# qq456cvb/VoteNet

Measured on AMD Instinct MI355X. Metric: SUN RGB-D 20k-pt scenes/sec (fwd+bwd), higher is better.
Workload: dtype f32

## Files before the change

votenet_amd/csrc/pool_bwd.hip:

```cpp
#include "mlp_types.h"
#include <mutex>
#include <set>

namespace votenet {

bool wgrad_fast_launch(int mode, const MlpIn &d, long rows, int cin, int cout, const float *dz, const BnSrc &bs, int bsrc, float *dw,
                       hipStream_t st, float *scratch);
void wgrad_reduce(int nslice, long pstride, long e0, long e1, const float *part, float *dw, hipStream_t st);

static inline int pb_grid(long total, int block, int cap)
{
    long g = (total + block - 1) / block;
    if (g > cap) g = cap;
    return (int)(g < 1 ? 1 : g);
}

__global__ __launch_bounds__(256) void bn_bwd_reduce_zsel_kernel(long groups, int c, const float *__restrict__ gout,
                                                                 const float *__restrict__ zsel, const float *__restrict__ scale,
                                                                 const float *__restrict__ shift, const float *__restrict__ mean,
                                                                 const float *__restrict__ var, float eps, int relu,
                                                                 double *__restrict__ sums, CoefTail tail)
{
    __shared__ float sh1[4][64], sh2[4][64];
    const int cx = threadIdx.x & 63, ry = threadIdx.x >> 6;
// ... 738 lines not shown
        for (int d = 0; d < D; d++) {
            if (c0 + (long)d * stride >= G) break;
            const long c = c0 + team + (long)d * stride;
            const bool live = c < G;
            float(*xt)[K][LD] = xs[buf];
            bool kept[NP];
#pragma unroll
            for (int j = 0; j < NP; j++) {
                kept[j] = n_row[d][j] >= 0;
                if (!kept[j]) continue;
#pragma unroll
                for (int h = 0; h < NL; h++) {
                    float4 v = nxt[d][j][h];
                    v.x = fmaxf(v.x * sc.x + sh.x, fl);
                    v.y = fmaxf(v.y * sc.y + sh.y, fl);
                    v.z = fmaxf(v.z * sc.z + sh.z, fl);
                    v.w = fmaxf(v.w * sc.w + sh.w, fl);
                    *reinterpret_cast<float4 *>(&xt[j][(tid + h * 256) / Q][q * 4]) = v;
                }
            }
            float gg = live ? n_g[d] : 0.0f;
            const float zz = n_z[d], w31 = n_w[d];
            const int ar = n_a[d];
            const long cn = c + (long)D * stride;
            fetch(d, cn < G ? cn : (live ? c : G - 1));
            __syncthreads();
            if (own) {
                if (relu && !(zz * cS + cH > 0.0f)) gg = 0.0f;
                const float v = cA * gg;
                const int pj = ar >> 4;
                const bool there = pj == 0 ? kept[0] : pj == 1 ? kept[1] : pj == 2 ? kept[2] : kept[3];
                if (v != 0.0f && there) {
                    const float4 *row = reinterpret_cast<const float4 *>(&xt[pj][ar & (K - 1)][0]);
#pragma unroll
                    for (int i0 = 0; i0 < Q; i0 += 8) {
                        float4 a[8];
#pragma unroll
                        for (int i = 0; i < 8; i++) a[i] = row[i0 + i];
                        asm volatile("" ::: "memory");
#pragma unroll
                        for (int i = 0; i < 8; i++) {
                            acc[4 * (i0 + i)] += a[i].x * v;
                            acc[4 * (i0 + i) + 1] += a[i].y * v;
                            acc[4 * (i0 + i) + 2] += a[i].z * v;
                            acc[4 * (i0 + i) + 3] += a[i].w * v;
                        }
                    }
                }
            }
            if (live && tid >= 256 - CIN) {
                const int jc = tid - (256 - CIN);
#pragma unroll
                for (int j = 0; j < NP; j++) {
                    if (!kept[j]) continue;
#pragma unroll 8
                    for (int r = (j == 0 ? 1 : 0); r < K; r++) csum += xt[j][r][jc];
                }
                csum += w31 * xt[0][0][jc];
            }
            buf ^= 1;
        }
    }
    if (TEAMS > 1) {
        __syncthreads();
        float *comb = sparse_smem;
        if (team == 1) {
            if (own) {
#pragma unroll
                for (int i = 0; i < CIN; i++) comb[(size_t)i * cout + tid] = acc[i];
            }
            if (tid >= 256 - CIN) comb[(size_t)CIN * cout + tid - (256 - CIN)] = csum;
        }
        __syncthreads();
        if (team == 1) return;
        if (own) {
#pragma unroll
            for (int i = 0; i < CIN; i++) acc[i] += comb[(size_t)i * cout + tid];
        }
        if (tid >= 256 - CIN) csum += comb[(size_t)CIN * cout + tid - (256 - CIN)];
    }
    if (own) {
#pragma unroll
        for (int i = 0; i < CIN; i++) unsafeAtomicAdd(&dw[(size_t)i * cout + tid], acc[i]);
    }
    if (tid >= 256 - CIN) unsafeAtomicAdd(&colsum[tid - (256 - CIN)], csum);
}

__global__ __launch_bounds__(256) void pool_wgrad_finish_kernel(int cin, int cout, const float *__restrict__ gram,
                                                                const float *__restrict__ colsum, const float *__restrict__ w,
                                                                const float *__restrict__ bias, const float *__restrict__ coef,
                                                                float *__restrict__ dw)
{
    __shared__ float Gs[16][33], Ws[32][17];
    const int tx = threadIdx.x & 15, ty = threadIdx.x >> 4;
    const int j0 = blockIdx.y * 16, c0 = blockIdx.x * 16;
    float acc = 0.0f;
    for (int i0 = 0; i0 < cin; i0 += 32) {
        for (int e = threadIdx.x; e < 16 * 32; e += 256) {
            const int r = e >> 5, ii = e & 31;
            Gs[r][ii] = (j0 + r < cin && i0 + ii < cin) ? gram[(size_t)(j0 + r) * cin + i0 + ii] : 0.0f;
            const int wr = e >> 4, wc = e & 15;
            Ws[wr][wc] = (i0 + wr < cin && c0 + wc < cout) ? w[(size_t)(i0 + wr) * cout + c0 + wc] : 0.0f;
        }
        __syncthreads();
#pragma unroll 8
        for (int ii = 0; ii < 32; ii++) acc += Gs[ty][ii] * Ws[ii][tx];
        __syncthreads();
    }
    const int j = j0 + ty, c = c0 + tx;
    if (j < cin && c < cout) {
        const float Cc = coef[2 * cout + c];
        dw[(size_t)j * cout + c] += Cc * acc + colsum[j] * (coef[cout + c] + Cc * (bias ? bias[c] : 0.0f));
    }
}

}

using namespace votenet;

extern "C" int votenet_pool_backward_supported(int cin, int cout, int k)
{
    return k == 64 && ((cin == 128 && (cout == 256 || cout == 128)) || (cin == 64 && cout == 128));
}

static int g_zsel_groups = 32, g_zsel_cap = 256;
extern "C" void votenet_debug_zsel_grid(int groups_per_wg, int cap)
{
    VN_DEBUG_GATE();
    g_zsel_groups = groups_per_wg > 0 ? groups_per_wg : 32;
    g_zsel_cap = cap > 0 ? cap : 256;
}
extern "C" int votenet_bn_backward_reduce_pool(long groups, int c, const float *gout, const float *zsel, const float *scale,
                                               const float *shift, const float *mean, const float *var, float eps, int relu,
                                               double *sums, const votenet_coef_tail *tail, void *stream)
{
    VN_REQUIRE(groups > 0 && c > 0, "bn_backward_reduce_pool expects groups > 0, c > 0");
    VN_REQUIRE(gout && zsel && scale && shift && mean && var && sums, "bn_backward_reduce_pool: null buffer");
    VN_REQUIRE(!tail || (tail->ticket && tail->gamma && tail->coef && tail->rows > 0), "bn_backward_reduce_pool: incomplete coefficient tail");
    const int ny = (c + 63) / 64;
    hipLaunchKernelGGL(bn_bwd_reduce_zsel_kernel, dim3(pb_grid(groups, g_zsel_groups, g_zsel_cap / ny), ny), dim3(256), 0, as_stream(stream), groups,
                       c, gout, zsel, scale, shift, mean, var, eps, relu, sums, to_tail(tail));
    return check_launch("bn_backward_reduce_pool");
}

static int pool_dgrad_prepare_launch(int cin, int cout, const float *w, const float *bias, const float *coef, float *mmat, float *cvec,
                                     void *image, void *stream, float *h2_ascale = nullptr, float *h2_unscale = nullptr)
{
    VN_REQUIRE(cin > 0 && w && coef && mmat && cvec, "pool_dgrad_prepare: bad arguments");
    VN_REQUIRE((cout == 128 || cout == 256) && (uintptr_t)w % 16 == 0, "pool_dgrad_prepare: cout must be 128 or 256 (got %d), w 16-byte aligned", cout);
    VN_REQUIRE(image == nullptr || (cin % 16 == 0 && (uintptr_t)image % 16 == 0), "pool_dgrad_prepare_split: cin %% 16 == 0 and a 16-byte aligned image");
    const dim3 grid((cin + 15) / 16, (cin + 15) / 16);
    unsigned *img = static_cast<unsigned *>(image);
    if (cout == 256)
        hipLaunchKernelGGL(pool_dgrad_prepare_kernel<256>, grid, dim3(256), 0, as_stream(stream), cin, w, bias, coef, mmat, cvec, img, h2_ascale, h2_unscale);
    else
        hipLaunchKernelGGL(pool_dgrad_prepare_kernel<128>, grid, dim3(256), 0, as_stream(stream), cin, w, bias, coef, mmat, cvec, img, h2_ascale, h2_unscale);
    return check_launch("pool_dgrad_prepare");
}
extern "C" int votenet_pool_dgrad_prepare(int cin, int cout, const float *w, const float *bias, const float *coef, float *mmat,
                                          float *cvec, void *stream)
{
    return pool_dgrad_prepare_launch(cin, cout, w, bias, coef, mmat, cvec, nullptr, stream);
}
extern "C" int votenet_pool_dgrad_prepare_h2(int cin, int cout, const float *w, const float *bias, const float *coef, float *mmat,
                                             float *cvec, void *image, float *ascale, float *unscale, void *stream)
{
    VN_REQUIRE(image != nullptr && ascale != nullptr && unscale != nullptr, "pool_dgrad_prepare_h2: null image / scale vectors");
    return pool_dgrad_prepare_launch(cin, cout, w, bias, coef, mmat, cvec, image, stream, ascale, unscale);
}
extern "C" int votenet_pool_dgrad_prepare_split(int cin, int cout, const float *w, const float *bias, const float *coef, float *mmat,
                                                float *cvec, void *image, void *stream)
{
    VN_REQUIRE(image != nullptr, "pool_dgrad_prepare_split: null image");
    return pool_dgrad_prepare_launch(cin, cout, w, bias, coef, mmat, cvec, image, stream);
}

static int g_scatter_reverse = 0;
extern "C" void votenet_debug_scatter_reverse(int on) { VN_DEBUG_GATE(); g_scatter_reverse = on ? 1 : 0; }
static int g_scatter_nwv = 16;
extern "C" void votenet_debug_scatter_waves(int n) { VN_DEBUG_GATE(); g_scatter_nwv = n == 12 ? 12 : 16; }
static int g_scatter_wgs = 0;
extern "C" void votenet_debug_scatter_workgroups(int n) { VN_DEBUG_GATE(); g_scatter_wgs = n > 0 ? n : 0; }
static int g_scatter_form = 1;
extern "C" void votenet_debug_scatter_form(int form) { VN_DEBUG_GATE(); g_scatter_form = form ? 1 : 0; }
static int pool_dgrad_scatter_launch(long groups, int k, int cin, int cout, const float *gout, const int *argmax, const float *zsel,
                                     const float *coef, int relu, const float *wT, float *da, const float *below_z,
                                     const float *below_scale, const float *below_shift, const float *below_mean, const float *below_var,
                                     float eps, int below_relu, double *below_sums, const votenet_coef_tail *below_tail, const int *hc,
                                     const float *wh, int G, void *stream, const int *nh_dev = nullptr);
extern "C" int votenet_pool_dgrad_scatter(long groups, int k, int cin, int cout, const float *gout, const int *argmax,
                                          const float *zsel, const float *coef, int relu, const float *wT, float *da,
                                          const float *below_z, const float *below_scale, const float *below_shift,
                                          const float *below_mean, const float *below_var, float eps, int below_relu,
                                          double *below_sums, const votenet_coef_tail *below_tail, void *stream)
{
    VN_REQUIRE(!below_tail || (below_z && below_tail->ticket && below_tail->gamma && below_tail->coef && below_tail->rows > 0),
               "pool_dgrad_scatter: incomplete coefficient tail");
    VN_REQUIRE(groups > 0 && gout && argmax && zsel && coef && wT && da, "pool_dgrad_scatter: bad arguments");
    VN_REQUIRE(votenet_pool_backward_supported(cin, cout, k), "pool_dgrad_scatter: unsupported shape cin=%d cout=%d k=%d", cin, cout, k);
    VN_REQUIRE((uintptr_t)wT % 16 == 0, "pool_dgrad_scatter: wT must be 16-byte aligned");
    VN_REQUIRE(!below_z || (below_scale && below_shift && below_mean && below_var && below_sums),
               "pool_dgrad_scatter: below_z given without the layer's BatchNorm vectors / sums");
    return pool_dgrad_scatter_launch(groups, k, cin, cout, gout, argmax, zsel, coef, relu, wT, da, below_z, below_scale, below_shift, below_mean,
                                     below_var, eps, below_relu, below_sums, below_tail, nullptr, nullptr, 0, stream);
}

extern "C" int votenet_pool_dgrad_scatter_half(long nh, int G, int cin, int cout, const float *gout, const int *argmax, const float *zsel,
                                               const float *coef, int relu, const float *wT, float *da, const int *hc, const float *wh,
                                               const float *below_z, const float *below_scale, const float *below_shift,
                                               const float *below_mean, const float *below_var, float eps, int below_relu,
                                               double *below_sums, const votenet_coef_tail *below_tail, const int *nh_dev, void *stream)
{
    VN_REQUIRE(hc && wh && G > 0 && nh >= G && nh <= (long)kBallPieces * G, "pool_dgrad_scatter_half: bad piece-layout arguments");
    VN_REQUIRE(gout && argmax && zsel && coef && wT && da && (uintptr_t)wT % 16 == 0, "pool_dgrad_scatter_half: null / unaligned buffer");
    VN_REQUIRE(votenet_pool_backward_supported(cin, cout, 64), "pool_dgrad_scatter_half: unsupported shape cin=%d cout=%d", cin, cout);
    VN_REQUIRE(!below_z || (below_scale && below_shift && below_mean && below_var && below_sums),
               "pool_dgrad_scatter_half: below_z given without the layer's BatchNorm vectors / sums");
    VN_REQUIRE(!below_tail || (below_z && below_tail->ticket && below_tail->gamma && below_tail->coef && below_tail->rows > 0),
               "pool_dgrad_scatter_half: incomplete coefficient tail");
    return pool_dgrad_scatter_launch(nh, 64, cin, cout, gout, argmax, zsel, coef, relu, wT, da, below_z, below_scale, below_shift, below_mean,
                                     below_var, eps, below_relu, below_sums, below_tail, hc, wh, G, stream, nh_dev);
}

static int pool_dgrad_scatter_launch(long groups, int k, int cin, int cout, const float *gout, const int *argmax, const float *zsel,
                                     const float *coef, int relu, const float *wT, float *da, const float *below_z,
                                     const float *below_scale, const float *below_shift, const float *below_mean, const float *below_var,
                                     float eps, int below_relu, double *below_sums, const votenet_coef_tail *below_tail, const int *hc,
                                     const float *wh, int G, void *stream, const int *nh_dev)
{
    hipStream_t st = as_stream(stream);
    const PoolBelow pb = {below_z, below_scale, below_shift, below_mean, below_var, eps, below_relu, below_sums, to_tail(below_tail), g_scatter_reverse, hc, wh, G, nh_dev};
    auto go = [&](auto kern, int ci, int co, int threads = 512) {
        const size_t smem = ((size_t)co * ci + 4 * co + 4 * k) * 4;
        const int per_cu = smem > 80 * 1024 ? 1 : (smem > 40 * 1024 ? 2 : 4);
        static std::set<const void *> raised;
        static std::mutex raised_mu;
        bool fresh;
        {
            std::lock_guard<std::mutex> lock(raised_mu);
            fresh = raised.insert(reinterpret_cast<const void *>(kern)).second;
        }
        if (fresh)
            (void)hipFuncSetAttribute(reinterpret_cast<const void *>(kern), hipFuncAttributeMaxDynamicSharedMemorySize, (int)smem);
        hipLaunchKernelGGL(kern, dim3(pb_grid(groups, 2, 256 * per_cu)), dim3(threads), smem, st, groups, gout, argmax, zsel, coef, relu,
                           wT, da, pb);
    };
    auto gow = [&](auto kern, int ci, int co, int kk, int nwv) {
        const size_t smem = (size_t)co * ci * 4 + (size_t)nwv * ((co + 3 * kk) * 6 + kk * 4);
        const int per_cu = smem > 80 * 1024 ? 1 : (smem > 40 * 1024 ? 2 : 4);
        static std::set<const void *> raised_w;
        static std::mutex raised_w_mu;
        bool fresh;
        {
            std::lock_guard<std::mutex> lock(raised_w_mu);
            fresh = raised_w.insert(reinterpret_cast<const void *>(kern)).second;
        }
        if (fresh)
            (void)hipFuncSetAttribute(reinterpret_cast<const void *>(kern), hipFuncAttributeMaxDynamicSharedMemorySize, (int)smem);
        hipLaunchKernelGGL(kern, dim3(pb_grid(groups, nwv, g_scatter_wgs > 0 ? g_scatter_wgs : 256 * per_cu)), dim3(nwv * 64), smem, st, groups, gout,
                           argmax, zsel, coef, relu, wT, da, pb);
    };
    if (g_scatter_form == 1 || hc) {
#define VN_SCATTER_WAVE(CI, CO, KK, NW)                                                            \
    do {                                                                                           \
        if (below_z) gow(pool_dgrad_scatter_wave_kernel<CI, CO, KK, true, NW>, CI, CO, KK, NW);   \
        else gow(pool_dgrad_scatter_wave_kernel<CI, CO, KK, false, NW>, CI, CO, KK, NW);          \
    } while (0)
        if (hc) {
            if (cin == 64) VN_SCATTER_WAVE(64, 128, kPiece, 8);
            else if (cout == 256) {
                if (g_scatter_nwv == 12) VN_SCATTER_WAVE(128, 256, kPiece, 12);
                else VN_SCATTER_WAVE(128, 256, kPiece, 16);
            }
            else VN_SCATTER_WAVE(128, 128, kPiece, 8);
        } else {
            if (cin == 64) VN_SCATTER_WAVE(64, 128, 64, 8);
            else if (cout == 256) VN_SCATTER_WAVE(128, 256, 64, 8);
            else VN_SCATTER_WAVE(128, 128, 64, 8);
        }
#undef VN_SCATTER_WAVE
        return check_launch("pool_dgrad_scatter");
    }
    if (below_z) {
        if (cin == 128 && cout == 256)
            go(pool_dgrad_scatter_kernel<128, 256, 64, true, 16>, 128, 256, 1024);
        else if (cin == 128)
            go(pool_dgrad_scatter_kernel<128, 128, 64, true>, 128, 128);
        else
            go(pool_dgrad_scatter_kernel<64, 128, 64, true>, 64, 128);
    } else {
        if (cin == 128 && cout == 256)
            go(pool_dgrad_scatter_kernel<128, 256, 64, false, 16>, 128, 256, 1024);
        else if (cin == 128)
            go(pool_dgrad_scatter_kernel<128, 128, 64, false>, 128, 128);
        else
            go(pool_dgrad_scatter_kernel<64, 128, 64, false>, 64, 128);
    }
    return check_launch("pool_dgrad_scatter");
}

#ifndef GRAM_ABL
#define GRAM_ABL 0
#endif
template <int C, int NP = 3>
__global__ __launch_bounds__(256) void gram_bf3_kernel(long rows, const float *__restrict__ x, const float *__restrict__ scale_shift,
                                                       int relu, float *__restrict__ gram, long rows_per_block,
                                                       const float *__restrict__ wh ,
                                                       const int *__restrict__ nh_dev )
{
    if (nh_dev != nullptr) {
        const long lim = (long)nh_dev[0] * kPiece;
        rows = lim < rows ? lim : rows;
    }
    constexpr int KPT = C / 16;
    constexpr int T = C / 64;
    constexpr int PL = C * 4 + 16;
    static_assert(NP == 2 || NP == 3, "pieces per operand");
    constexpr float kA = NP == 2 ? 16.0f : 1.0f, kUn = NP == 2 ? 1.0f / 256.0f : 1.0f;
    __shared__ __attribute__((aligned(16))) unsigned Ts[2][NP][2][PL];
    const int tid = threadIdx.x, lane = tid & 63;
    const int wv = __builtin_amdgcn_readfirstlane(tid >> 6);
    const int wi = wv >> 1, wj = wv & 1;
    const long r_begin = (long)blockIdx.x * rows_per_block;
    if (r_begin >= rows) return;
    const int nrow = (int)((r_begin + rows_per_block < rows ? r_begin + rows_per_block : rows) - r_begin);
    const int nslab = (nrow + 15) / 16;
    const int c = tid % C, rg = tid / C;
    const int kh_w = (C == 128) ? rg : (rg >> 1), d_w = (C == 128) ? 0 : (rg & 1) * 2;
    const float sc = scale_shift[c] * kA, sh = scale_shift[C + c] * kA;
    const float floor_ = relu ? 0.0f : -__builtin_inff();
    const float *xb = x + (size_t)r_begin * C + c;
    float R[2][KPT];
    static_assert(kPiece == 16, "one slab = one piece");
    const bool first_rg = rg == 0;
    const float *whb = wh ? wh + r_begin / kPiece : nullptr;
    const float *whp = whb ? whb : scale_shift;
    float Wq[2] = {1.0f, 1.0f};
    bool abl_prologue = true;
    auto load = [&](float (&r)[KPT], int s, float &wq) {
        if ((GRAM_ABL & 4) && !abl_prologue) return;
#pragma unroll
        for (int i = 0; i < KPT; i++) {
            int lr = s * 16 + rg * KPT + i;
            lr = lr < nrow ? lr : nrow - 1;
            r[i] = xb[(size_t)lr * C];
        }
        const int sw = (whb != nullptr && s * 16 < nrow) ? s : 0;
        wq = whp[sw];
    };
    auto store = [&](int buf, const float (&r)[KPT], int s, float wq) {
        if ((GRAM_ABL & 8) && !abl_prologue) return;
        float v[KPT];
#pragma unroll
        for (int i = 0; i < KPT; i++) {
            v[i] = fmaxf(r[i] * sc + sh, floor_);
            if (s * 16 + rg * KPT + i >= nrow) v[i] = 0.0f;
        }
        if (whb != nullptr && first_rg && s * 16 < nrow) v[0] *= sqrtf(wq);
        if constexpr (NP == 2) {
            unsigned h[KPT / 2], l[KPT / 2];
#pragma unroll
            for (int i = 0; i < KPT / 2; i++) split2(v[2 * i], v[2 * i + 1], h[i], l[i]);
            if constexpr (C == 128) {
                *reinterpret_cast<uint4 *>(&Ts[buf][0][kh_w][c * 4]) = make_uint4(h[0], h[1], h[2], h[3]);
                *reinterpret_cast<uint4 *>(&Ts[buf][1][kh_w][c * 4]) = make_uint4(l[0], l[1], l[2], l[3]);
            } else {
                *reinterpret_cast<uint2 *>(&Ts[buf][0][kh_w][c * 4 + d_w]) = make_uint2(h[0], h[1]);
                *reinterpret_cast<uint2 *>(&Ts[buf][1][kh_w][c * 4 + d_w]) = make_uint2(l[0], l[1]);
            }
            return;
        }
        unsigned h[KPT / 2], m[KPT / 2], l[KPT / 2];
#pragma unroll
        for (int i = 0; i < KPT / 2; i++) split3(v[2 * i], v[2 * i + 1], h[i], m[i], l[i]);
        if constexpr (C == 128) {
            *reinterpret_cast<uint4 *>(&Ts[buf][0][kh_w][c * 4]) = make_uint4(h[0], h[1], h[2], h[3]);
            *reinterpret_cast<uint4 *>(&Ts[buf][1][kh_w][c * 4]) = make_uint4(m[0], m[1], m[2], m[3]);
            *reinterpret_cast<uint4 *>(&Ts[buf][NP - 1][kh_w][c * 4]) = make_uint4(l[0], l[1], l[2], l[3]);
        } else {
            *reinterpret_cast<uint2 *>(&Ts[buf][0][kh_w][c * 4 + d_w]) = make_uint2(h[0], h[1]);
            *reinterpret_cast<uint2 *>(&Ts[buf][1][kh_w][c * 4 + d_w]) = make_uint2(m[0], m[1]);
            *reinterpret_cast<uint2 *>(&Ts[buf][NP - 1][kh_w][c * 4 + d_w]) = make_uint2(l[0], l[1]);
        }
    };
    f32x16 acc[T][T];
#pragma unroll
    for (int a = 0; a < T; a++)
#pragma unroll
        for (int b = 0; b < T; b++)
#pragma unroll
            for (int e = 0; e < 16; e++) acc[a][b][e] = 0.0f;
    load(R[0], 0, Wq[0]);
    store(0, R[0], 0, Wq[0]);
    load(R[1], 1, Wq[1]);
    __builtin_amdgcn_sched_barrier(0);
    load(R[0], 2, Wq[0]);
    __syncthreads();
    const int kh = lane >> 5, l31 = lane & 31;
    int buf = 0;
    abl_prologue = false;
    const int nslab2 = (nslab + 1) & ~1;
    for (int s = 0; s < nslab2; s += 2) {
#pragma unroll
        for (int par = 0; par < 2; par++) {
            uint4 fa[NP][T], fb[NP][T];
#pragma unroll
            for (int p = 0; p < NP; p++) {
#pragma unroll
                for (int t = 0; t < T; t++) {
                    fa[p][t] = *reinterpret_cast<const uint4 *>(&Ts[buf][p][kh][((wi * T + t) * 32 + l31) * 4]);
                    fb[p][t] = *reinterpret_cast<const uint4 *>(&Ts[buf][p][kh][((wj * T + t) * 32 + l31) * 4]);
                }
            }
            auto mm = [&](int pa, int pb) {
                if (GRAM_ABL & 1) {
                    acc[0][0][0] += __uint_as_float(fa[pa][0].x ^ fb[pb][0].y);
                    return;
                }
#pragma unroll
                for (int a = 0; a < T; a++)
#pragma unroll
                    for (int b = 0; b < T; b++) {
                        if constexpr (NP == 2)
                            acc[a][b] = __builtin_amdgcn_mfma_f32_32x32x16_f16(__builtin_bit_cast(f16x8, fa[pa][a]),
                                                                               __builtin_bit_cast(f16x8, fb[pb][b]), acc[a][b], 0, 0, 0);
                        else
                            acc[a][b] = __builtin_amdgcn_mfma_f32_32x32x16_bf16(__builtin_bit_cast(bf16x8, fa[pa][a]),
                                                                                __builtin_bit_cast(bf16x8, fb[pb][b]), acc[a][b], 0, 0, 0);
                    }
            };
            if constexpr (NP == 2) {
                mm(1, 0);
                mm(0, 1);
                store(buf ^ 1, R[par ^ 1], s + par + 1, Wq[par ^ 1]);
                load(R[par ^ 1], s + par + 3, Wq[par ^ 1]);
                mm(0, 0);
            } else {
                mm(2, 0);
                mm(0, 2);
                mm(1, 1);
                store(buf ^ 1, R[par ^ 1], s + par + 1, Wq[par ^ 1]);
                load(R[par ^ 1], s + par + 3, Wq[par ^ 1]);
                mm(1, 0);
                mm(0, 1);
                mm(0, 0);
            }
            lds_barrier();
            buf ^= 1;
        }
    }
    if (GRAM_ABL & 2) {
        float t_ = 0.0f;
#pragma unroll
        for (int a = 0; a < T; a++)
#pragma unroll
            for (int b = 0; b < T; b++)
#pragma unroll
                for (int e = 0; e < 16; e++) t_ += acc[a][b][e];
        if (t_ == 12345.678f) gram[0] = t_;
        return;
    }
#pragma unroll
    for (int a = 0; a < T; a++)
#pragma unroll
        for (int b = 0; b < T; b++) {
            const int j = (wj * T + b) * 32 + l31;
#pragma unroll
            for (int e = 0; e < 16; e++) {
                const int i = (wi * T + a) * 32 + (e & 3) + 8 * (e >> 2) + 4 * kh;
                unsafeAtomicAdd(&gram[(size_t)i * C + j], acc[a][b][e] * kUn);
            }
        }
}

int g_gram_bf3 = 1;
static int g_gram_wgs = 384;
template <int C>
static void gram_bf3_launch(long rows, const float *z, const float *scale_shift, int relu, float *gram, hipStream_t st, const float *wh = nullptr,
                            const int *nh_dev = nullptr)
{
    long rpb = (rows + g_gram_wgs - 1) / g_gram_wgs;
    rpb = (rpb + 31) / 32 * 32;
    if (rpb < 128) rpb = 128;
    const unsigned gx = (unsigned)((rows + rpb - 1) / rpb);
    if (g_gram_bf3 != 3) hipLaunchKernelGGL((gram_bf3_kernel<C, 2>), dim3(gx), dim3(256), 0, st, rows, z, scale_shift, relu, gram, rpb, wh, nh_dev);
    else hipLaunchKernelGGL((gram_bf3_kernel<C, 3>), dim3(gx), dim3(256), 0, st, rows, z, scale_shift, relu, gram, rpb, wh, nh_dev);
}
extern "C" void votenet_debug_gram_bf3(int on) { VN_DEBUG_GATE(); g_gram_bf3 = on; }
extern "C" void votenet_debug_gram_workgroups(int n) { VN_DEBUG_GATE(); g_gram_wgs = n > 0 ? n : 384; }

extern "C" int votenet_mlp_gram(long rows, int c, const float *z, const float *scale_shift, int relu, float *gram, float *scratch,
                                void *stream)
{
    if (g_gram_bf3 && scratch == nullptr && (c == 64 || c == 128) && rows > 0 && rows < (1L << 31) / c && z && scale_shift && gram &&
        (uintptr_t)z % 16 == 0) {
        if (c == 128) gram_bf3_launch<128>(rows, z, scale_shift, relu, gram, as_stream(stream));
        else gram_bf3_launch<64>(rows, z, scale_shift, relu, gram, as_stream(stream));
        return check_launch("mlp_gram");
    }
    VN_REQUIRE(rows > 0 && c > 0 && z && scale_shift && gram, "mlp_gram: bad arguments");
    MlpIn d = {};
    d.x = z;
    d.in_scale = scale_shift;
    d.in_shift = scale_shift + c;
    d.in_relu = relu;
    BnSrc bs = {};
    bs.z = z;
    bs.coef = scale_shift;
    bs.relu = relu;
    VN_REQUIRE(wgrad_fast_launch(0, d, rows, c, c, nullptr, bs, 3, gram, as_stream(stream), scratch),
               "mlp_gram: shape not served (c %% 64 == 0, 16-byte aligned operands), got c = %d", c);
    return check_launch("mlp_gram");
}

static int g_sparse_wgs = 384, g_sparse_wgs2 = 256, g_sparse_teams = 2;
extern "C" void votenet_debug_sparse_workgroups(int n) { VN_DEBUG_GATE(); g_sparse_wgs = n > 0 ? n : 384; }
extern "C" void votenet_debug_sparse_teams(int teams, int wgs)
{
    VN_DEBUG_GATE();
    g_sparse_teams = teams == 1 ? 1 : 2;
    if (wgs > 0) g_sparse_wgs2 = wgs;
}
static int pool_wgrad_sparse_launch(long groups, int cin, int cout, const float *xz, const float *in_scale, const float *in_shift, int in_relu,
                                    const float *gout, const int *argmax, const float *zsel, const float *coef, int relu, float *dw,
                                    float *colsum, float *scratch, const int *hc, const float *wh, int G, void *stream, const int *nh_dev = nullptr);
extern "C" int votenet_pool_wgrad_sparse(long groups, int k, int cin, int cout, const float *xz, const float *in_scale,
                                         const float *in_shift, int in_relu, const float *gout, const int *argmax, const float *zsel,
                                         const float *coef, int relu, float *dw, float *colsum, float *scratch, void *stream)
{
    VN_REQUIRE(groups > 0 && xz && gout && argmax && zsel && coef && dw && colsum, "pool_wgrad_sparse: bad arguments");
    VN_REQUIRE(cin <= cout, "pool_wgrad_sparse expects cin <= cout");
    VN_REQUIRE(votenet_pool_backward_supported(cin, cout, k), "pool_wgrad_sparse: unsupported shape cin=%d cout=%d k=%d", cin, cout, k);
    VN_REQUIRE((in_scale == nullptr) == (in_shift == nullptr), "pool_wgrad_sparse: in_scale and in_shift go together");
    VN_REQUIRE((uintptr_t)xz % 16 == 0 && (!in_scale || ((uintptr_t)in_scale % 16 == 0 && (uintptr_t)in_shift % 16 == 0)),
               "pool_wgrad_sparse: operands must be 16-byte aligned");
    return pool_wgrad_sparse_launch(groups, cin, cout, xz, in_scale, in_shift, in_relu, gout, argmax, zsel, coef, relu, dw, colsum, scratch,
                                    nullptr, nullptr, 0, stream);
}

extern "C" int votenet_mlp_gram_half(long rows, int c, const float *z, const float *scale_shift, int relu, const float *wh, float *gram,
                                     const int *nh_dev, void *stream)
{
    VN_REQUIRE(rows > 0 && rows % kPiece == 0 && rows < (1L << 31) / c && (c == 128 || c == 64), "mlp_gram_half expects rows %% 16 == 0 and c in {64, 128}");
    VN_REQUIRE(z && scale_shift && wh && gram && (uintptr_t)z % 16 == 0, "mlp_gram_half: null / unaligned buffer");
    if (c == 128) gram_bf3_launch<128>(rows, z, scale_shift, relu, gram, as_stream(stream), wh, nh_dev);
    else gram_bf3_launch<64>(rows, z, scale_shift, relu, gram, as_stream(stream), wh, nh_dev);
    return check_launch("mlp_gram_half");
}

extern "C" int votenet_pool_wgrad_sparse_half(long nh, int G, int cin, int cout, const float *xz, const float *in_scale, const float *in_shift,
                                              int in_relu, const float *gout, const int *argmax, const float *zsel, const float *coef, int relu,
                                              float *dw, float *colsum, const int *hc, const float *wh, const int *nh_dev, void *stream)
{
    VN_REQUIRE(nh > 0 && G > 0 && nh >= G && nh <= (long)kBallPieces * G && hc && wh, "pool_wgrad_sparse_half: bad piece-layout arguments");
    VN_REQUIRE(xz && gout && argmax && zsel && coef && dw && colsum, "pool_wgrad_sparse_half: bad arguments");
    VN_REQUIRE(votenet_pool_backward_supported(cin, cout, 64), "pool_wgrad_sparse_half: unsupported shape cin=%d cout=%d", cin, cout);
    VN_REQUIRE((in_scale == nullptr) == (in_shift == nullptr), "pool_wgrad_sparse_half: in_scale and in_shift go together");
    VN_REQUIRE((uintptr_t)xz % 16 == 0 && (!in_scale || ((uintptr_t)in_scale % 16 == 0 && (uintptr_t)in_shift % 16 == 0)),
               "pool_wgrad_sparse_half: operands must be 16-byte aligned");
    return pool_wgrad_sparse_launch(nh, cin, cout, xz, in_scale, in_shift, in_relu, gout, argmax, zsel, coef, relu, dw, colsum, nullptr, hc, wh,
                                    G, stream, nh_dev);
}

static int g_sparse_centre_wgs = 192, g_sparse_centre_teams = 2;
extern "C" void votenet_debug_sparse_centre_workgroups(int n) { VN_DEBUG_GATE(); g_sparse_centre_wgs = n > 0 ? n : 192; }
extern "C" void votenet_debug_sparse_centre_teams(int t) { VN_DEBUG_GATE(); g_sparse_centre_teams = t == 1 ? 1 : 2; }
extern "C" int votenet_pool_wgrad_sparse_half_centres(long nh, int G, int cin, int cout, const float *xz, const float *in_scale,
                                                      const float *in_shift, int in_relu, const float *gout, const int *argmax,
                                                      const float *zsel, const float *coef, int relu, float *dw, float *colsum,
                                                      const int *pos, const float *wh, const int *nh_dev, void *stream)
{
    VN_REQUIRE(nh > 0 && G > 0 && nh >= G && nh <= (long)kBallPieces * G && pos && wh, "pool_wgrad_sparse_half_centres: bad piece-layout arguments");
    VN_REQUIRE(xz && gout && argmax && zsel && coef && dw && colsum, "pool_wgrad_sparse_half_centres: bad arguments");
    VN_REQUIRE(votenet_pool_backward_supported(cin, cout, 64), "pool_wgrad_sparse_half_centres: unsupported shape cin=%d cout=%d", cin, cout);
    VN_REQUIRE((in_scale == nullptr) == (in_shift == nullptr), "pool_wgrad_sparse_half_centres: in_scale and in_shift go together");
    VN_REQUIRE((size_t)nh * kPiece * (size_t)cin * 4 < ((size_t)1 << 31),
               "pool_wgrad_sparse_half_centres: nh*16*cin*4 = %zu bytes exceeds the 2 GiB the centre-walking kernel addresses; "
               "use votenet_pool_wgrad_sparse_half", (size_t)nh * kPiece * (size_t)cin * 4);
    VN_REQUIRE((uintptr_t)xz % 16 == 0 && (!in_scale || ((uintptr_t)in_scale % 16 == 0 && (uintptr_t)in_shift % 16 == 0)),
               "pool_wgrad_sparse_half_centres: operands must be 16-byte aligned");
    hipStream_t st = as_stream(stream);
    const int teams = g_sparse_centre_teams;
    auto go = [&](auto kern, int ci) {
        const size_t tiles = (size_t)teams * 2 * kBallPieces * kPiece * (ci + 4) * 4;
        const size_t comb = teams > 1 ? (size_t)(ci + 1) * cout * 4 : 0;
        const size_t smem = tiles > comb ? tiles : comb;
        static std::set<const void *> raised_c;
        static std::mutex raised_c_mu;
        bool fresh;
        {
            std::lock_guard<std::mutex> lock(raised_c_mu);
            fresh = raised_c.insert(reinterpret_cast<const void *>(kern)).second;
        }
        if (fresh) (void)hipFuncSetAttribute(reinterpret_cast<const void *>(kern), hipFuncAttributeMaxDynamicSharedMemorySize, (int)smem);
        const int grid = pb_grid(G, 8 * teams, g_sparse_centre_wgs * 2 / teams);
        hipLaunchKernelGGL(kern, dim3(grid), dim3(256 * teams), smem, st, G, nh, cout, xz, in_scale, in_shift, in_relu, gout, argmax, zsel, coef, relu, dw,
                           colsum, pos, wh, nh_dev);
    };
    if (teams == 1) {
        if (cin == 64) go(pool_wgrad_sparse_centre_kernel<64, 1>, 64);
        else go(pool_wgrad_sparse_centre_kernel<128, 1>, 128);
    } else if (cin == 64) go(pool_wgrad_sparse_centre_kernel<64, 2>, 64);
    else go(pool_wgrad_sparse_centre_kernel<128, 2>, 128);
    return check_launch("pool_wgrad_sparse_half_centres");
}

static int pool_wgrad_sparse_launch(long groups, int cin, int cout, const float *xz, const float *in_scale, const float *in_shift, int in_relu,
                                    const float *gout, const int *argmax, const float *zsel, const float *coef, int relu, float *dw,
                                    float *colsum, float *scratch, const int *hc, const float *wh, int G, void *stream, const int *nh_dev)
{
    hipStream_t st = as_stream(stream);
    int grid;
    auto go = [&](auto kern, int ci, int kk, int teams, int cap) {
        const size_t tiles = (size_t)teams * (kk == kPiece ? 2 : 1) * kk * (ci + 4) * 4;
        const size_t comb = teams > 1 ? (size_t)(ci + 1) * cout * 4 : 0;
        const size_t smem = tiles > comb ? tiles : comb;
        static std::set<const void *> raised_s;
        static std::mutex raised_s_mu;
        bool fresh;
        {
            std::lock_guard<std::mutex> lock(raised_s_mu);
            fresh = raised_s.insert(reinterpret_cast<const void *>(kern)).second;
        }
        if (fresh) (void)hipFuncSetAttribute(reinterpret_cast<const void *>(kern), hipFuncAttributeMaxDynamicSharedMemorySize, (int)smem);
        grid = pb_grid(groups, (kk == kPiece ? 32 : 8) * teams, cap);
        hipLaunchKernelGGL(kern, dim3(grid), dim3(256 * teams), smem, st, groups, cout, xz, in_scale, in_shift, in_relu, gout, argmax, zsel, coef,
                           relu, dw, colsum, scratch, hc, wh, G, nh_dev);
    };
    if (hc && g_sparse_teams == 2 && !scratch) {
        if (cin == 64) go(pool_wgrad_sparse_kernel<64, kPiece, 2>, 64, kPiece, 2, g_sparse_wgs2);
        else go(pool_wgrad_sparse_kernel<128, kPiece, 2>, 128, kPiece, 2, g_sparse_wgs2);
    } else if (hc) {
        if (cin == 64) go(pool_wgrad_sparse_kernel<64, kPiece, 1>, 64, kPiece, 1, g_sparse_wgs);
        else go(pool_wgrad_sparse_kernel<128, kPiece, 1>, 128, kPiece, 1, g_sparse_wgs);
    } else if (cin == 128) {
        go(pool_wgrad_sparse_kernel<128, 64, 1>, 128, 64, 1, g_sparse_wgs);
    } else {
        go(pool_wgrad_sparse_kernel<64, 64, 1>, 64, 64, 1, g_sparse_wgs);
    }
    if (scratch) {
        const long ps = (long)(cin + 1) * cout;
        wgrad_reduce(grid, ps, 0, (long)cin * cout, scratch, dw, st);
        wgrad_reduce(grid, ps, (long)cin * cout, (long)cin * cout + cin, scratch, colsum - (long)cin * cout, st);
    }
    return check_launch("pool_wgrad_sparse");
}

extern "C" size_t votenet_pool_wgrad_scratch_floats(long groups, int cin, int cout)
{
    if (groups <= 0) return 0;
    return (size_t)pb_grid(groups, 8, g_sparse_wgs) * (size_t)(cin + 1) * cout;
}

extern "C" int votenet_pool_wgrad_finish(int cin, int cout, const float *gram, const float *colsum, const float *w, const float *bias,
                                         const float *coef, float *dw, void *stream)
{
    VN_REQUIRE(cin > 0 && cout > 0 && gram && colsum && w && coef && dw, "pool_wgrad_finish: bad arguments");
    hipLaunchKernelGGL(pool_wgrad_finish_kernel, dim3((cout + 15) / 16, (cin + 15) / 16), dim3(256), 0, as_stream(stream), cin, cout,
                       gram, colsum, w, bias, coef, dw);
    return check_launch("pool_wgrad_finish");
}
```

Measured before the change: 2281.

## Exploit Gram symmetry with upper-triangle MFMA tiles and two-group workgroups

```diff
diff --git a/votenet_amd/csrc/pool_bwd.hip b/votenet_amd/csrc/pool_bwd.hip
--- a/votenet_amd/csrc/pool_bwd.hip
+++ b/votenet_amd/csrc/pool_bwd.hip
@@ -1064,50 +1064,77 @@
 #ifndef GRAM_ABL
 #define GRAM_ABL 0
 #endif
-template <int C, int NP = 3>
-__global__ __launch_bounds__(256) void gram_bf3_kernel(long rows, const float *__restrict__ x, const float *__restrict__ scale_shift,
-                                                       int relu, float *__restrict__ gram, long rows_per_block,
-                                                       const float *__restrict__ wh ,
-                                                       const int *__restrict__ nh_dev )
+struct GramDeal {
+    int nf, nt;
+    int a[3], b[3];
+};
+constexpr GramDeal kGramDeal[5] = {
+    {2, 3, {0, 0, 1}, {0, 1, 1}},
+    {3, 2, {0, 0, 0}, {1, 2, 0}},
+    {1, 1, {0, 0, 0}, {0, 0, 0}},
+    {2, 1, {0, 0, 0}, {1, 0, 0}},
+    {0, 0, {0, 0, 0}, {0, 0, 0}},
+};
+template <int M>
+struct GramMode {
+    static constexpr int value = M;
+};
+template <int C, int NP = 3, int NG = 1>
+__global__ __launch_bounds__(256 * NG) void gram_bf3_kernel(long rows, const float *__restrict__ x, const float *__restrict__ scale_shift,
+                                                            int relu, float *__restrict__ gram, long rows_per_group,
+                                                            const float *__restrict__ wh ,
+                                                            const int *__restrict__ nh_dev )
 {
     if (nh_dev != nullptr) {
         const long lim = (long)nh_dev[0] * kPiece;
         rows = lim < rows ? lim : rows;
     }
-    constexpr int KPT = C / 16;
-    constexpr int T = C / 64;
+    constexpr int KPT = 8;
+    constexpr int SUB = 128 / C;
+    constexpr int SR = 16 * SUB;
     constexpr int PL = C * 4 + 16;
+    constexpr int NTG = C == 128 ? 10 : 3;
+    constexpr int TP = 32 * 33;
     static_assert(NP == 2 || NP == 3, "pieces per operand");
+    static_assert(C == 64 || C == 128, "two or four sub-tile rows");
+    static_assert(NG == 1 || NG == 2, "groups of four waves per workgroup");
     constexpr float kA = NP == 2 ? 16.0f : 1.0f, kUn = NP == 2 ? 1.0f / 256.0f : 1.0f;
-    __shared__ __attribute__((aligned(16))) unsigned Ts[2][NP][2][PL];
-    const int tid = threadIdx.x, lane = tid & 63;
-    const int wv = __builtin_amdgcn_readfirstlane(tid >> 6);
-    const int wi = wv >> 1, wj = wv & 1;
-    const long r_begin = (long)blockIdx.x * rows_per_block;
-    if (r_begin >= rows) return;
-    const int nrow = (int)((r_begin + rows_per_block < rows ? r_begin + rows_per_block : rows) - r_begin);
-    const int nslab = (nrow + 15) / 16;
-    const int c = tid % C, rg = tid / C;
-    const int kh_w = (C == 128) ? rg : (rg >> 1), d_w = (C == 128) ? 0 : (rg & 1) * 2;
+    constexpr int TS_DW = NG * 2 * NP * SUB * 2 * PL, EP_DW = 4 * TP + (NG - 1) * NTG * 1024;
+    __shared__ __attribute__((aligned(16))) unsigned smem[TS_DW > EP_DW ? TS_DW : EP_DW];
+    const int tid = threadIdx.x, lane = tid & 63, lt = tid & 255;
+    const int wvg = __builtin_amdgcn_readfirstlane(tid >> 6);
+    const int grp = wvg >> 2, wv = wvg & 3;
+    auto Ts = [&](int buf, int p, int sub, int kh) -> unsigned * { return smem + ((((grp * 2 + buf) * NP + p) * SUB + sub) * 2 + kh) * PL; };
+    const long r_wg = (long)blockIdx.x * NG * rows_per_group;
+    if (r_wg >= rows) return;
+    const int nslab = (int)(((r_wg + rows_per_group < rows ? rows_per_group : rows - r_wg) + SR - 1) / SR);
+    const long r_begin = r_wg + (long)grp * rows_per_group;
+    const int nrow = r_begin >= rows ? 0 : (int)((r_begin + rows_per_group < rows ? r_begin + rows_per_group : rows) - r_begin);
+    const long r_base = nrow > 0 ? r_begin : 0;
+    const int last = nrow > 0 ? nrow - 1 : 0;
+    const int c = lt % C, rg = lt / C;
+    const int sub_w = rg >> 1, kh_w = rg & 1;
     const float sc = scale_shift[c] * kA, sh = scale_shift[C + c] * kA;
     const float floor_ = relu ? 0.0f : -__builtin_inff();
-    const float *xb = x + (size_t)r_begin * C + c;
-    float R[2][KPT];
+    const float *xb = x + (size_t)r_base * C + c;
+    constexpr int NSET = 2;
+    float R[NSET][KPT];
     static_assert(kPiece == 16, "one slab = one piece");
-    const bool first_rg = rg == 0;
-    const float *whb = wh ? wh + r_begin / kPiece : nullptr;
+    const bool first_rg = kh_w == 0;
+    const float *whb = wh ? wh + r_base / kPiece : nullptr;
     const float *whp = whb ? whb : scale_shift;
-    float Wq[2] = {1.0f, 1.0f};
+    float Wq[NSET] = {1.0f, 1.0f};
     bool abl_prologue = true;
     auto load = [&](float (&r)[KPT], int s, float &wq) {
         if ((GRAM_ABL & 4) && !abl_prologue) return;
 #pragma unroll
         for (int i = 0; i < KPT; i++) {
-            int lr = s * 16 + rg * KPT + i;
-            lr = lr < nrow ? lr : nrow - 1;
+            int lr = s * SR + rg * KPT + i;
+            lr = lr < nrow ? lr : last;
             r[i] = xb[(size_t)lr * C];
         }
-        const int sw = (whb != nullptr && s * 16 < nrow) ? s : 0;
+        const int q = s * SUB + sub_w;
+        const int sw = (whb != nullptr && q * 16 < nrow) ? q : 0;
         wq = whp[sw];
     };
     auto store = [&](int buf, const float (&r)[KPT], int s, float wq) {
@@ -1116,140 +1143,184 @@
 #pragma unroll
         for (int i = 0; i < KPT; i++) {
             v[i] = fmaxf(r[i] * sc + sh, floor_);
-            if (s * 16 + rg * KPT + i >= nrow) v[i] = 0.0f;
-        }
-        if (whb != nullptr && first_rg && s * 16 < nrow) v[0] *= sqrtf(wq);
+            if (s * SR + rg * KPT + i >= nrow) v[i] = 0.0f;
+        }
+        if (whb != nullptr && first_rg && (s * SUB + sub_w) * 16 < nrow) v[0] *= sqrtf(wq);
         if constexpr (NP == 2) {
             unsigned h[KPT / 2], l[KPT / 2];
 #pragma unroll
             for (int i = 0; i < KPT / 2; i++) split2(v[2 * i], v[2 * i + 1], h[i], l[i]);
-            if constexpr (C == 128) {
-                *reinterpret_cast<uint4 *>(&Ts[buf][0][kh_w][c * 4]) = make_uint4(h[0], h[1], h[2], h[3]);
-                *reinterpret_cast<uint4 *>(&Ts[buf][1][kh_w][c * 4]) = make_uint4(l[0], l[1], l[2], l[3]);
-            } else {
-                *reinterpret_cast<uint2 *>(&Ts[buf][0][kh_w][c * 4 + d_w]) = make_uint2(h[0], h[1]);
-                *reinterpret_cast<uint2 *>(&Ts[buf][1][kh_w][c * 4 + d_w]) = make_uint2(l[0], l[1]);
-            }
+            *reinterpret_cast<uint4 *>(Ts(buf, 0, sub_w, kh_w) + c * 4) = make_uint4(h[0], h[1], h[2], h[3]);
+            *reinterpret_cast<uint4 *>(Ts(buf, 1, sub_w, kh_w) + c * 4) = make_uint4(l[0], l[1], l[2], l[3]);
             return;
         }
         unsigned h[KPT / 2], m[KPT / 2], l[KPT / 2];
 #pragma unroll
         for (int i = 0; i < KPT / 2; i++) split3(v[2 * i], v[2 * i + 1], h[i], m[i], l[i]);
-        if constexpr (C == 128) {
-            *reinterpret_cast<uint4 *>(&Ts[buf][0][kh_w][c * 4]) = make_uint4(h[0], h[1], h[2], h[3]);
-            *reinterpret_cast<uint4 *>(&Ts[buf][1][kh_w][c * 4]) = make_uint4(m[0], m[1], m[2], m[3]);
-            *reinterpret_cast<uint4 *>(&Ts[buf][NP - 1][kh_w][c * 4]) = make_uint4(l[0], l[1], l[2], l[3]);
-        } else {
-            *reinterpret_cast<uint2 *>(&Ts[buf][0][kh_w][c * 4 + d_w]) = make_uint2(h[0], h[1]);
-            *reinterpret_cast<uint2 *>(&Ts[buf][1][kh_w][c * 4 + d_w]) = make_uint2(m[0], m[1]);
-            *reinterpret_cast<uint2 *>(&Ts[buf][NP - 1][kh_w][c * 4 + d_w]) = make_uint2(l[0], l[1]);
-        }
+        *reinterpret_cast<uint4 *>(Ts(buf, 0, sub_w, kh_w) + c * 4) = make_uint4(h[0], h[1], h[2], h[3]);
+        *reinterpret_cast<uint4 *>(Ts(buf, 1, sub_w, kh_w) + c * 4) = make_uint4(m[0], m[1], m[2], m[3]);
+        *reinterpret_cast<uint4 *>(Ts(buf, NP - 1, sub_w, kh_w) + c * 4) = make_uint4(l[0], l[1], l[2], l[3]);
     };
-    f32x16 acc[T][T];
-#pragma unroll
-    for (int a = 0; a < T; a++)
-#pragma unroll
-        for (int b = 0; b < T; b++)
-#pragma unroll
-            for (int e = 0; e < 16; e++) acc[a][b][e] = 0.0f;
     load(R[0], 0, Wq[0]);
     store(0, R[0], 0, Wq[0]);
-    load(R[1], 1, Wq[1]);
     __builtin_amdgcn_sched_barrier(0);
-    load(R[0], 2, Wq[0]);
+#pragma unroll
+    for (int j = 1; j < NSET; j++) load(R[j], j, Wq[j]);
+    load(R[0], NSET, Wq[0]);
     __syncthreads();
     const int kh = lane >> 5, l31 = lane & 31;
-    int buf = 0;
     abl_prologue = false;
-    const int nslab2 = (nslab + 1) & ~1;
-    for (int s = 0; s < nslab2; s += 2) {
-#pragma unroll
-        for (int par = 0; par < 2; par++) {
-            uint4 fa[NP][T], fb[NP][T];
-#pragma unroll
-            for (int p = 0; p < NP; p++) {
-#pragma unroll
-                for (int t = 0; t < T; t++) {
-                    fa[p][t] = *reinterpret_cast<const uint4 *>(&Ts[buf][p][kh][((wi * T + t) * 32 + l31) * 4]);
-                    fb[p][t] = *reinterpret_cast<const uint4 *>(&Ts[buf][p][kh][((wj * T + t) * 32 + l31) * 4]);
+    const int nslabn = (nslab + NSET - 1) / NSET * NSET;
+    auto run = [&](auto mode) {
+        constexpr GramDeal D = kGramDeal[decltype(mode)::value];
+        constexpr int NF = D.nf, NT = D.nt;
+        int xr[3] = {0, 0, 0};
+        if constexpr (decltype(mode)::value == 0) xr[0] = 2 * wv, xr[1] = 2 * wv + 1;
+        if constexpr (decltype(mode)::value == 1) xr[0] = wv - 2, xr[1] = 2, xr[2] = 3;
+        if constexpr (decltype(mode)::value == 2) xr[0] = wv;
+        if constexpr (decltype(mode)::value == 3) xr[1] = 1;
+        f32x16 acc[NT > 0 ? NT : 1];
+#pragma unroll
+        for (int t = 0; t < NT; t++)
+#pragma unroll
+            for (int e = 0; e < 16; e++) acc[t][e] = 0.0f;
+        int buf = 0;
+        for (int s = 0; s < nslabn; s += NSET) {
+#pragma unroll
+            for (int par = 0; par < NSET; par++) {
+                const int nx = (par + 1) % NSET;
+                uint4 f[SUB][NP][NF > 0 ? NF : 1];
+#pragma unroll
+                for (int u = 0; u < SUB; u++)
+#pragma unroll
+                    for (int p = 0; p < NP; p++)
+#pragma unroll
+                        for (int q = 0; q < NF; q++) f[u][p][q] = *reinterpret_cast<const uint4 *>(Ts(buf, p, u, kh) + (xr[q] * 32 + l31) * 4);
+                auto mm = [&](int pa, int pb) {
+                    if (GRAM_ABL & 1) {
+                        if constexpr (NT > 0) acc[0][0] += __uint_as_float(f[0][pa][0].x ^ f[0][pb][0].y);
+                        return;
+                    }
+#pragma unroll
+                    for (int u = 0; u < SUB; u++)
+#pragma unroll
+                        for (int t = 0; t < NT; t++) {
+                            if constexpr (NP == 2)
+                                acc[t] = __builtin_amdgcn_mfma_f32_32x32x16_f16(__builtin_bit_cast(f16x8, f[u][pa][D.a[t]]),
+                                                                                __builtin_bit_cast(f16x8, f[u][pb][D.b[t]]), acc[t], 0, 0, 0);
+                            else
+                                acc[t] = __builtin_amdgcn_mfma_f32_32x32x16_bf16(__builtin_bit_cast(bf16x8, f[u][pa][D.a[t]]),
+                                                                                 __builtin_bit_cast(bf16x8, f[u][pb][D.b[t]]), acc[t], 0, 0, 0);
+                        }
+                };
+                if constexpr (NP == 2) {
+                    mm(1, 0);
+                    mm(0, 1);
+                    store(buf ^ 1, R[nx], s + par + 1, Wq[nx]);
+                    load(R[nx], s + par + 1 + NSET, Wq[nx]);
+                    mm(0, 0);
+                } else {
+                    mm(2, 0);
+                    mm(0, 2);
+                    mm(1, 1);
+                    store(buf ^ 1, R[nx], s + par + 1, Wq[nx]);
+                    load(R[nx], s + par + 1 + NSET, Wq[nx]);
+                    mm(1, 0);
+                    mm(0, 1);
+                    mm(0, 0);
                 }
-            }
-            auto mm = [&](int pa, int pb) {
-                if (GRAM_ABL & 1) {
-                    acc[0][0][0] += __uint_as_float(fa[pa][0].x ^ fb[pb][0].y);
-                    return;
-                }
-#pragma unroll
-                for (int a = 0; a < T; a++)
-#pragma unroll
-                    for (int b = 0; b < T; b++) {
-                        if constexpr (NP == 2)
-                            acc[a][b] = __builtin_amdgcn_mfma_f32_32x32x16_f16(__builtin_bit_cast(f16x8, fa[pa][a]),
-                                                                               __builtin_bit_cast(f16x8, fb[pb][b]), acc[a][b], 0, 0, 0);
-                        else
-                            acc[a][b] = __builtin_amdgcn_mfma_f32_32x32x16_bf16(__builtin_bit_cast(bf16x8, fa[pa][a]),
-                                                                                __builtin_bit_cast(bf16x8, fb[pb][b]), acc[a][b], 0, 0, 0);
-                    }
-            };
-            if constexpr (NP == 2) {
-                mm(1, 0);
-                mm(0, 1);
-                store(buf ^ 1, R[par ^ 1], s + par + 1, Wq[par ^ 1]);
-                load(R[par ^ 1], s + par + 3, Wq[par ^ 1]);
-                mm(0, 0);
-            } else {
-                mm(2, 0);
-                mm(0, 2);
-                mm(1, 1);
-                store(buf ^ 1, R[par ^ 1], s + par + 1, Wq[par ^ 1]);
-                load(R[par ^ 1], s + par + 3, Wq[par ^ 1]);
-                mm(1, 0);
-                mm(0, 1);
-                mm(0, 0);
-            }
-            lds_barrier();
-            buf ^= 1;
-        }
-    }
-    if (GRAM_ABL & 2) {
-        float t_ = 0.0f;
-#pragma unroll
-        for (int a = 0; a < T; a++)
-#pragma unroll
-            for (int b = 0; b < T; b++)
-#pragma unroll
-                for (int e = 0; e < 16; e++) t_ += acc[a][b][e];
-        if (t_ == 12345.678f) gram[0] = t_;
-        return;
-    }
-#pragma unroll
-    for (int a = 0; a < T; a++)
-#pragma unroll
-        for (int b = 0; b < T; b++) {
-            const int j = (wj * T + b) * 32 + l31;
+                lds_barrier();
+                buf ^= 1;
+            }
+        }
+        if (GRAM_ABL & 2) {
+            float t_ = 0.0f;
+#pragma unroll
+            for (int t = 0; t < NT; t++)
+#pragma unroll
+                for (int e = 0; e < 16; e++) t_ += acc[t][e];
+            if (t_ == 12345.678f) gram[0] = t_;
+            return;
+        }
+        float *ep = reinterpret_cast<float *>(smem);
+        if constexpr (NG == 2) {
+            float *cb = ep + 4 * TP + (C == 128 ? (wv < 2 ? 3 * wv : 2 + 2 * wv) : wv) * 1024;
+            if (grp == 1) {
+#pragma unroll
+                for (int t = 0; t < NT; t++)
+#pragma unroll
+                    for (int e = 0; e < 16; e++) cb[t * 1024 + e * 64 + lane] = acc[t][e];
+            }
+            __syncthreads();
+            if (grp == 1) return;
+#pragma unroll
+            for (int t = 0; t < NT; t++)
+#pragma unroll
+                for (int e = 0; e < 16; e++) acc[t][e] += cb[t * 1024 + e * 64 + lane];
+        }
+        float *tp = ep + wv * TP;
+#pragma unroll
+        for (int t = 0; t < NT; t++) {
+            const int ti = xr[D.a[t]], tj = xr[D.b[t]];
+            const bool diag = D.a[t] == D.b[t];
 #pragma unroll
             for (int e = 0; e < 16; e++) {
-                const int i = (wi * T + a) * 32 + (e & 3) + 8 * (e >> 2) + 4 * kh;
-                unsafeAtomicAdd(&gram[(size_t)i * C + j], acc[a][b][e] * kUn);
-            }
-        }
+                const int li = (e & 3) + 8 * (e >> 2) + 4 * kh;
+                const float v = acc[t][e] * kUn;
+                if (!diag || li <= l31) unsafeAtomicAdd(&gram[(size_t)(ti * 32 + li) * C + tj * 32 + l31], v);
+                tp[li * 33 + l31] = v;
+            }
+            __builtin_amdgcn_wave_barrier();
+            asm volatile("s_waitcnt lgkmcnt(0)" ::: "memory");
+#pragma unroll
+            for (int e = 0; e < 16; e++) {
+                const int lj = (e & 3) + 8 * (e >> 2) + 4 * kh;
+                const float v = tp[l31 * 33 + lj];
+                if (!diag || l31 < lj) unsafeAtomicAdd(&gram[(size_t)(tj * 32 + lj) * C + ti * 32 + l31], v);
+            }
+            __builtin_amdgcn_wave_barrier();
+            asm volatile("s_waitcnt lgkmcnt(0)" ::: "memory");
+        }
+    };
+    if constexpr (C == 128) {
+        if (wv < 2) run(GramMode<0>{});
+        else run(GramMode<1>{});
+    } else {
+        if (wv < 2) run(GramMode<2>{});
+        else if (wv == 2) run(GramMode<3>{});
+        else run(GramMode<4>{});
+    }
 }
 
 int g_gram_bf3 = 1;
-static int g_gram_wgs = 384;
+static int g_gram_wgs = 0;
+static int g_gram_groups = 2;
 template <int C>
 static void gram_bf3_launch(long rows, const float *z, const float *scale_shift, int relu, float *gram, hipStream_t st, const float *wh = nullptr,
                             const int *nh_dev = nullptr)
 {
-    long rpb = (rows + g_gram_wgs - 1) / g_gram_wgs;
-    rpb = (rpb + 31) / 32 * 32;
-    if (rpb < 128) rpb = 128;
-    const unsigned gx = (unsigned)((rows + rpb - 1) / rpb);
-    if (g_gram_bf3 != 3) hipLaunchKernelGGL((gram_bf3_kernel<C, 2>), dim3(gx), dim3(256), 0, st, rows, z, scale_shift, relu, gram, rpb, wh, nh_dev);
-    else hipLaunchKernelGGL((gram_bf3_kernel<C, 3>), dim3(gx), dim3(256), 0, st, rows, z, scale_shift, relu, gram, rpb, wh, nh_dev);
+    const int ng = g_gram_groups;
+    const int wgs = g_gram_wgs > 0 ? g_gram_wgs : nh_dev != nullptr ? 384 : C == 64 ? 256 : 192;
+    const long vw = (long)wgs * ng;
+    long rpg = (rows + vw - 1) / vw;
+    rpg = (rpg + 31) / 32 * 32;
+    if (rpg < 128) rpg = 128;
+    const unsigned gx = (unsigned)((rows + rpg * ng - 1) / (rpg * ng));
+    if (ng == 2) {
+        if (g_gram_bf3 != 3) hipLaunchKernelGGL((gram_bf3_kernel<C, 2, 2>), dim3(gx), dim3(512), 0, st, rows, z, scale_shift, relu, gram, rpg, wh, nh_dev);
+        else hipLaunchKernelGGL((gram_bf3_kernel<C, 3, 2>), dim3(gx), dim3(512), 0, st, rows, z, scale_shift, relu, gram, rpg, wh, nh_dev);
+    } else {
+        if (g_gram_bf3 != 3) hipLaunchKernelGGL((gram_bf3_kernel<C, 2, 1>), dim3(gx), dim3(256), 0, st, rows, z, scale_shift, relu, gram, rpg, wh, nh_dev);
+        else hipLaunchKernelGGL((gram_bf3_kernel<C, 3, 1>), dim3(gx), dim3(256), 0, st, rows, z, scale_shift, relu, gram, rpg, wh, nh_dev);
+    }
 }
 extern "C" void votenet_debug_gram_bf3(int on) { VN_DEBUG_GATE(); g_gram_bf3 = on; }
-extern "C" void votenet_debug_gram_workgroups(int n) { VN_DEBUG_GATE(); g_gram_wgs = n > 0 ? n : 384; }
+extern "C" void votenet_debug_gram_workgroups(int n)
+{
+    VN_DEBUG_GATE();
+    g_gram_wgs = n > 0 ? n : -n;
+    g_gram_groups = n < 0 ? 1 : 2;
+}
 
 extern "C" int votenet_mlp_gram(long rows, int c, const float *z, const float *scale_shift, int relu, float *gram, float *scratch,
                                 void *stream)
```

After: 2299 (median of 6 runs). No clear change (+0.8%).
